# ariloytynoja/pagan2-msa

Measured on AMD Instinct MI355X. Metric: DP cells/sec, 32x100 kb DNA progressive align (hot path in dependency order: fill + traceback per tree level), higher is better.
Workload: dtype f64; 1 GPU; cfg4_32x100kb_dna_anchored; leaves=32, length=100000, data_type=dna, anchors=prefix, offset 15, node_alignments=31, order=guide-tree levels one after the other (a parent needs its children)

## Files before the change

include/pagan_dp.h:

```cpp
#ifndef PAGAN_DP_H
#define PAGAN_DP_H

#include <stdint.h>

#ifdef __cplusplus
extern "C" {
#endif

#define PAGAN_OK              0
#define PAGAN_E_ARG          -1
#define PAGAN_E_GRAPH        -2
#define PAGAN_E_BAND         -3
#define PAGAN_E_MODEL        -4
#define PAGAN_E_NODEVICE     -5
#define PAGAN_E_NOMEM        -6
#define PAGAN_E_INTERNAL     -7
#define PAGAN_DP_REACHED      0
#define PAGAN_DP_UNREACHABLE  1

#define PAGAN_OPT_NO_TERMINAL_EDGES        1u
#define PAGAN_OPT_NO_REDUCED_TERMINAL_PEN  2u

enum { PAGAN_X_MAT = 0, PAGAN_Y_MAT = 1, PAGAN_M_MAT = 2 };
enum { PAGAN_MATCHED = 2, PAGAN_XGAPPED = 3, PAGAN_YGAPPED = 4,
// ... 99 lines not shown
int  pagan_dp_debug_strips(const pagan_graph *left, const pagan_graph *right, const pagan_band *band, int32_t max_sites,
                           int32_t *strips , int32_t cap, int64_t *desc_off ,
                           int64_t *desc , int64_t desc_cap);
int  pagan_dp_debug_tiles(const pagan_graph *left, const pagan_graph *right, const pagan_band *band,
                          int32_t *tiles , int32_t cap, int32_t *tile_side);
int  pagan_dp_debug_tiles_staircase(const int32_t *tiles, int32_t n);
int  pagan_dp_debug_compact(const pagan_graph *left, const pagan_graph *right, const pagan_band *band, int32_t *keep_left,
                            int32_t *keep_right, int32_t *slot_left, int32_t *slot_right, int32_t *upper, int32_t *lower,
                            int32_t *n_out);
int  pagan_dp_debug_route(const pagan_graph *left, const pagan_graph *right, const pagan_model *model, const pagan_band *band,
                          int32_t *n_out);
int  pagan_batch_debug_scores(pagan_batch *b, int32_t k, double *dst, int64_t count);
int  pagan_batch_debug_backptrs(pagan_batch *b, int32_t k, uint32_t *dst, int64_t count);
int  pagan_batch_debug_poison(pagan_batch *b);
int  pagan_batch_debug_followed(pagan_batch *b, int32_t k, int32_t *counts);
int  pagan_batch_debug_poke_bp(pagan_batch *b, int32_t k, int32_t i, int32_t j, int32_t vit, uint32_t word);
int  pagan_batch_debug_reruns(pagan_batch *b);

void    pagan_dp_release_cache(void);
int64_t pagan_dp_cached_device_bytes(int32_t device);

typedef struct pagan_model_prob {
    int32_t      n_states;
    const float *score;
    float        gap_open;
    float        gap_ext;
    float        non_gap;
} pagan_model_prob;

typedef struct pagan_fb pagan_fb;
// ... 66 lines not shown
```

pagan2-msa_amd/__init__.py:

```python
import ctypes as C
import os

from . import abi
from .abi import Band, Graph, Model, ModelProb, Result

_HERE = os.path.dirname(os.path.abspath(__file__))
LIB_PATH = os.environ.get("PAGAN_DP_LIB") or os.path.join(_HERE, "libpagan_dp.so")
_lib = None


class PaganError(RuntimeError):
    def __init__(self, code, what):
        super().__init__("%s failed with code %d" % (what, code))
        self.code = code


def lib():
    global _lib
    if _lib is None:
        if not os.path.exists(LIB_PATH):
            raise RuntimeError("libpagan_dp.so is missing: run `python -c 'import __graft_entry__ as g; g.build()'`")
        _lib = abi.declare(C.CDLL(LIB_PATH))
    return _lib

# ... 514 lines not shown
               "pagan_batch_debug_scores")
        return out

    def debug_backptrs(self, k):
        import numpy as np
        out = np.empty((self.cells_of(k), 3), np.uint32)
        _check(self._L.pagan_batch_debug_backptrs(self._h, k, out.ctypes.data_as(C.POINTER(C.c_uint32)), out.size),
               "pagan_batch_debug_backptrs")
        return out

    def debug_followed(self, k):
        c = (C.c_int32 * 2)()
        _check(self._L.pagan_batch_debug_followed(self._h, k, c), "pagan_batch_debug_followed")
        return int(c[0]), int(c[1])

    def debug_poke_bp(self, k, i, j, vit, word):
        _check(self._L.pagan_batch_debug_poke_bp(self._h, k, i, j, vit, word), "pagan_batch_debug_poke_bp")

    def debug_reruns(self):
        return int(self._L.pagan_batch_debug_reruns(self._h))

    def debug_trace(self, k, n_cells):
        import numpy as np
        out = np.empty((n_cells, 3), np.int32)
        _check(self._L.pagan_batch_debug_trace(self._h, k, out.ctypes.data_as(C.c_void_p), out.nbytes), "pagan_batch_debug_trace")
        return out

    def debug_segments(self, k):
        import numpy as np
        info = np.zeros(4, np.int32)
# ... 22 lines not shown
```

pagan2-msa_amd/abi.py:

```python
import ctypes as C

import numpy as np

PAGAN_OK = 0
PAGAN_E_ARG, PAGAN_E_GRAPH, PAGAN_E_BAND, PAGAN_E_MODEL = -1, -2, -3, -4
PAGAN_E_NODEVICE, PAGAN_E_NOMEM, PAGAN_E_INTERNAL = -5, -6, -7
PAGAN_DP_REACHED, PAGAN_DP_UNREACHABLE = 0, 1
OPT_NO_TERMINAL_EDGES = 1
OPT_NO_REDUCED_TERMINAL_PEN = 2
SAMPLE_NO_TRACES = 1
DECODE_KEEP_MATRIX = 1
X_MAT, Y_MAT, M_MAT = 0, 1, 2
MATCHED, XGAPPED, YGAPPED, XSKIPPED, YSKIPPED = 2, 3, 4, 5, 6

_i32p = C.POINTER(C.c_int32)
_f32p = C.POINTER(C.c_float)


class CGraph(C.Structure):
    _fields_ = [("n_sites", C.c_int32), ("n_edges", C.c_int32), ("state", _i32p), ("bwd_off", _i32p),
                ("bwd_src", _i32p), ("bwd_logw", _f32p), ("bwd_eid", _i32p)]


class CModel(C.Structure):
# ... 167 lines not shown
    lib.pagan_dp_debug_strips.restype = C.c_int
    lib.pagan_dp_debug_tiles.argtypes = [gp, gp, bp, _i32p, C.c_int32, _i32p]
    lib.pagan_dp_debug_tiles.restype = C.c_int
    lib.pagan_dp_debug_compact.argtypes = [gp, gp, bp, _i32p, _i32p, _i32p, _i32p, _i32p, _i32p, _i32p]
    lib.pagan_dp_debug_compact.restype = C.c_int
    lib.pagan_dp_debug_tiles_staircase.argtypes = [_i32p, C.c_int32]
    lib.pagan_dp_debug_tiles_staircase.restype = C.c_int
    lib.pagan_dp_debug_route.argtypes = [gp, gp, C.POINTER(CModel), bp, _i32p]
    lib.pagan_dp_debug_route.restype = C.c_int
    lib.pagan_batch_debug_scores.argtypes = [C.c_void_p, C.c_int32, C.POINTER(C.c_double), C.c_int64]
    lib.pagan_batch_debug_scores.restype = C.c_int
    lib.pagan_batch_debug_backptrs.argtypes = [C.c_void_p, C.c_int32, C.POINTER(C.c_uint32), C.c_int64]
    lib.pagan_batch_debug_backptrs.restype = C.c_int
    lib.pagan_batch_debug_followed.argtypes = [C.c_void_p, C.c_int32, C.POINTER(C.c_int32)]
    lib.pagan_batch_debug_followed.restype = C.c_int
    lib.pagan_batch_debug_poke_bp.argtypes = [C.c_void_p, C.c_int32, C.c_int32, C.c_int32, C.c_int32, C.c_uint32]
    lib.pagan_batch_debug_poke_bp.restype = C.c_int
    lib.pagan_batch_debug_reruns.argtypes = [C.c_void_p]
    lib.pagan_batch_debug_reruns.restype = C.c_int
    lib.pagan_batch_debug_poison.argtypes = [C.c_void_p]
    lib.pagan_batch_debug_poison.restype = C.c_int
    lib.pagan_dp_release_cache.argtypes = []
    lib.pagan_dp_release_cache.restype = None
    lib.pagan_dp_cached_device_bytes.argtypes = [C.c_int32]
    lib.pagan_dp_cached_device_bytes.restype = C.c_int64
    mpp, f64p = C.POINTER(CModelProb), C.POINTER(C.c_double)
    lib.pagan_fb_run.argtypes = [gp, gp, mpp, bp, op, C.POINTER(C.c_void_p)]
    lib.pagan_fb_run.restype = C.c_int
    lib.pagan_fb_run_batch.argtypes = [C.c_int32, C.POINTER(gp), C.POINTER(gp), C.POINTER(mpp), C.POINTER(bp), op, C.POINTER(C.c_void_p)]
    lib.pagan_fb_run_batch.restype = C.c_int
# ... 66 lines not shown
    lib.pagan_fb_debug_decode_route.restype = C.c_int
    lib.pagan_fb_decode_predict_bytes.argtypes = [C.c_int32, C.c_int32, bp]
    lib.pagan_fb_decode_predict_bytes.restype = C.c_int64
    lib.pagan_fb_decoded_destroy.argtypes = [C.c_void_p]
    lib.pagan_fb_decoded_destroy.restype = None
    lib.pagan_fb_destroy.argtypes = [C.c_void_p]
    lib.pagan_fb_destroy.restype = None
    lib.pagan_dp_version.argtypes = []
    lib.pagan_dp_version.restype = C.c_char_p
    return lib


EXPORTED = ["pagan_dp_align", "pagan_dp_align_batch", "pagan_result_free", "pagan_dp_predict_bytes",
            "pagan_dp_count_cells", "pagan_dp_device_count", "pagan_dp_select_device", "pagan_batch_create",
            "pagan_batch_run", "pagan_batch_sync", "pagan_batch_fetch", "pagan_batch_last_ms",
            "pagan_batch_cells", "pagan_batch_last_ms_detail", "pagan_batch_destroy", "pagan_batch_debug_trace", "pagan_batch_debug_segments", "pagan_dp_debug_plan", "pagan_dp_debug_far", "pagan_dp_debug_strips", "pagan_dp_debug_tiles", "pagan_dp_debug_compact", "pagan_dp_debug_tiles_staircase", "pagan_dp_release_cache", "pagan_dp_cached_device_bytes", "pagan_dp_debug_route", "pagan_batch_debug_scores", "pagan_batch_debug_backptrs", "pagan_batch_debug_poison", "pagan_batch_debug_followed", "pagan_batch_debug_poke_bp", "pagan_batch_debug_reruns",
            "pagan_fb_run", "pagan_fb_run_batch", "pagan_fb_totals", "pagan_fb_kernel_ms", "pagan_fb_groups", "pagan_fb_schedule", "pagan_fb_debug_route", "pagan_fb_dump", "pagan_fb_posterior_cells", "pagan_fb_sample_path",
            "pagan_path_cells", "pagan_fb_path_support", "pagan_fb_site_marginals", "pagan_fb_site_marginals_batch", "pagan_fb_post_ms", "pagan_fb_predict_bytes", "pagan_sample_uniforms",
            "pagan_sample_uniforms_path", "pagan_fb_sample_paths_batch", "pagan_fb_sample_paths", "pagan_fb_samples_summary", "pagan_fb_samples_visited",
            "pagan_fb_samples_visited_all", "pagan_fb_samples_result", "pagan_fb_samples_ms", "pagan_fb_sample_predict_bytes", "pagan_fb_samples_destroy",
            "pagan_fb_decode_batch", "pagan_fb_decode", "pagan_fb_decoded_summary", "pagan_fb_decoded_visited", "pagan_fb_decoded_result",
            "pagan_fb_decoded_dump", "pagan_fb_decoded_ms", "pagan_fb_debug_decode_route", "pagan_fb_decode_predict_bytes", "pagan_fb_decoded_destroy",
            "pagan_fb_destroy", "pagan_dp_version"]
```

pagan2-msa_amd/csrc/dp_abi.hip:

```cpp
#include <hip/hip_runtime.h>

#include <algorithm>
#include <atomic>
#include <thread>
#include <chrono>
#include <cmath>
#include <cstdint>
#include <cstdio>
#include <cstdlib>
#include <cstring>
#include <condition_variable>
#include <mutex>
#include <new>
#include <type_traits>
#include <vector>
#include <unordered_map>

#include "host_anchors.h"
#include "host_graph.h"
#include "../../include/pagan_dp.h"
#include "dp_device.h"
#include "dp_band.h"

template <int BLOCK> __global__ void pg_fill_wavefront(const PgDevJob *jobs, const int *which, unsigned flags);
// ... 966 lines not shown
    d->segs = c.take<int>(6 * (size_t)(2 * hj.n_bound + 8));
}
constexpr size_t kEndStride = 64;
void carve_ends(Carver &c, int n, PgDevJob *dj) {
    char *ends = c.take<char>(kEndStride * (size_t)n);
    for (int k = 0; k < n; ++k) {
        dj[k].endcell = reinterpret_cast<int *>(ends + kEndStride * (size_t)k);
        dj[k].endscore = reinterpret_cast<double *>(ends + kEndStride * (size_t)k + 32);
    }
}

void carve_follow(Carver &c, int n, const std::vector<HostJob> &jobs, PgDevJob *dj, size_t *begin, size_t *bytes) {
    *begin = (c.cur + 255) & ~(size_t)255;
    c.cur = *begin;
    for (int k = 0; k < n; ++k) {
        dj[k].follow = nullptr; dj[k].bp_done = nullptr;
        if (jobs[k].cls.empty()) continue;
        dj[k].follow = c.take<int>(4);
        dj[k].bp_done = c.take<unsigned char>((((size_t)dj[k].nd + PG_FOLLOW_CHUNK - 1) / PG_FOLLOW_CHUNK + 15) & ~(size_t)15);
    }
    *bytes = c.cur - *begin;
}

struct StagePool {
    std::mutex m;
    std::vector<std::pair<char *, size_t>> idle;
    char *take(size_t n, size_t *cap) {
        {
            std::lock_guard<std::mutex> g(m);
            for (size_t k = 0; k < idle.size(); ++k)
                if (idle[k].second >= n) {
                    char *p = idle[k].first; *cap = idle[k].second;
                    idle.erase(idle.begin() + k);
                    return p;
// ... 83 lines not shown
        static std::atomic<bool> lds_set_dev[64];
        std::atomic<bool> &lds_set = lds_set_dev[b->device & 63];
        if (!lds_set.load()) {
            HIP_TRY(hipFuncSetAttribute(reinterpret_cast<const void *>(pg_fill_ring<true>),
                                        hipFuncAttributeMaxDynamicSharedMemorySize, (int)pg_ring_lds_bytes()));
            HIP_TRY(hipFuncSetAttribute(reinterpret_cast<const void *>(pg_fill_ring<false>),
                                        hipFuncAttributeMaxDynamicSharedMemorySize, (int)pg_ring_lds_bytes()));
            lds_set.store(true);
        }
        const int n_small = b->n_ring_small, n_big = b->n_ring - b->n_ring_small;
        HIP_TRY(hipEventRecord(b->evk[0], b->stream)); b->evk_set[0] = true;
        if (b->use_pipe) {
            bool follow = b->bp_pass == 1 && b->follow_bytes > 0 && !b->no_follow;
            if (const char *f = std::getenv("PAGAN_DP_FOLLOW")) follow = follow && std::strcmp(f, "0") != 0;
            if (b->follow_bytes > 0) HIP_TRY(hipMemsetAsync(b->arena.dev + b->follow_begin, 0, b->follow_bytes, b->stream));
            auto followers = [&](int n_fill) { return follow && n_fill <= 32 ? std::min(96, 48 * ((n_fill + 7) / 8)) : 0; };
            if (n_small > 0)
                hipLaunchKernelGGL((pg_fill_pipe<true, false>), dim3(n_small + followers(n_small)), dim3(pg_pipe_block()), 0 , b->stream,
                                   b->d_jobs, b->d_which, b->flags | chk_banded, n_small);
            if (n_big > 0)
                hipLaunchKernelGGL((pg_fill_pipe<false, false>), dim3(n_big + followers(n_big)), dim3(pg_pipe_block()), 0, b->stream,
                                   b->d_jobs, b->d_which + n_small, b->flags | chk_banded, n_big);
            HIP_TRY(hipEventRecord(b->evk[1], b->stream)); b->evk_set[1] = true;
            if (b->bp_pass) {
                int max_nd = 1, max_w = 1;
                for (int k = 0; k < b->n; ++k) if (b->jobs[k].ring_ok) { max_nd = std::max(max_nd, b->dj[k].nd); max_w = std::max(max_w, b->jobs[k].dx.max_width); }
                const int zc = (max_w + PG_BP_CELLS - 1) / PG_BP_CELLS, dpb = bp_diags_per_block(max_nd, b->n_ring * zc);
                hipLaunchKernelGGL(pg_backptr, dim3((max_nd + dpb - 1) / dpb, b->n_ring, zc), dim3(256), 0, b->stream,
                                   b->d_jobs, b->d_which, (b->flags & 0xffu) | (b->bp_pass == 2 ? 0x100u : chk_banded), dpb);
                HIP_TRY(hipEventRecord(b->evk[2], b->stream)); b->evk_set[2] = true;
            }
        } else {
            b->evk_set[1] = false;
            if (n_small > 0)
                hipLaunchKernelGGL(pg_fill_ring<true>, dim3(n_small), dim3(576), pg_ring_lds_bytes(), b->stream,
                                   b->d_jobs, b->d_which, b->flags);
            if (n_big > 0)
// ... 688 lines not shown
    });
    const double tc3 = now();
    b->trace_off.resize(n); b->end_off.resize(n); b->score_off.resize(n);
    char *base = b->arena.dev;
    auto rebase = [&](auto *&p) { p = reinterpret_cast<std::remove_reference_t<decltype(p)>>(base + reinterpret_cast<size_t>(p)); };
    for (int k = 0; k < n; ++k) {
        PgDevJob &d = b->dj[k];
        b->trace_off[k] = reinterpret_cast<size_t>(d.trace);
        b->end_off[k] = reinterpret_cast<size_t>(d.endcell);
        b->score_off[k] = reinterpret_cast<size_t>(d.endscore);
        rebase(d.stL); rebase(d.offL); rebase(d.srcL); rebase(d.lwL);
        rebase(d.stR); rebase(d.offR); rebase(d.srcR); rebase(d.lwR);
        rebase(d.table); rebase(d.imin); rebase(d.imax); rebase(d.doff); rebase(d.tb); rebase(d.dsc); if (d.psc) { rebase(d.psc); rebase(d.sched); } if (d.hfL) { rebase(d.hfL); rebase(d.hfR); } rebase(d.fill_status);
        rebase(d.sc); rebase(d.bp);
        rebase(d.trace); rebase(d.endcell); rebase(d.endscore); rebase(d.segs); rebase(d.ttab);
        if (d.follow) { rebase(d.follow); rebase(d.bp_done); }
    }
    for (size_t g = 0; g < sdev.size(); ++g) {
        const StripPlan &sp = b->jobs[sdev[g].job].strips[sdev[g].q];
        PgDevJob d = b->dj[sdev[g].job];
        d.psc = reinterpret_cast<int *>(base + reinterpret_cast<size_t>(sdev[g].psc)) - 8 * (ptrdiff_t)sp.d0;
        d.sched = reinterpret_cast<int *>(base + reinterpret_cast<size_t>(sdev[g].sched));
        d.follow = reinterpret_cast<int *>(base + reinterpret_cast<size_t>(sdev[g].follow));
        d.bp_done = nullptr;
        d.nd = sp.d1;
        d.is_strip = 1; d.strip_row0 = sp.r0; d.d_first = sp.d0; d.feed_wave = sp.feed_wave; d.col_first = sp.col_first;
        d.pdsc = b->dj[sdev[g].job].dsc;
        d.prev_follow = nullptr; d.prev_nd = 0;
        if (sdev[g].q > 0) {
            d.prev_follow = b->dj[(size_t)n + g - 1].follow;
            d.prev_nd = b->dj[(size_t)n + g - 1].nd;
        }
        b->dj[(size_t)n + g] = d;
    }
    std::memcpy(stage.data() + reinterpret_cast<size_t>(jobs_off), b->dj.data(), sizeof(PgDevJob) * b->dj.size());
    std::memcpy(stage.data() + reinterpret_cast<size_t>(which_off), which_ring.data(), sizeof(int) * n);
    if (!swhich.empty()) std::memcpy(stage.data() + reinterpret_cast<size_t>(swhich_off), swhich.data(), sizeof(int) * swhich.size());
    b->d_swhich = reinterpret_cast<int *>(base + reinterpret_cast<size_t>(swhich_off));
    b->d_jobs = reinterpret_cast<PgDevJob *>(base + reinterpret_cast<size_t>(jobs_off));
// ... 243 lines not shown
int pagan_batch_debug_reruns(pagan_batch *b) { return b ? b->reruns : PAGAN_E_ARG; }

int pagan_batch_debug_followed(pagan_batch *b, int32_t k, int32_t *counts) {
    if (!b || k < 0 || k >= b->n || !counts) return PAGAN_E_ARG;
    counts[0] = counts[1] = 0;
    if (!b->dj[k].bp_done) return PAGAN_OK;
    HIP_TRY(hipStreamSynchronize(b->stream));
    const size_t n = ((size_t)b->dj[k].nd + PG_FOLLOW_CHUNK - 1) / PG_FOLLOW_CHUNK;
    std::vector<unsigned char> flags(n);
    HIP_TRY(hipMemcpy(flags.data(), b->dj[k].bp_done, n, hipMemcpyDeviceToHost));
    counts[1] = (int32_t)n;
    for (unsigned char f : flags) counts[0] += f != 0;
    return PAGAN_OK;
}

int pagan_batch_debug_scores(pagan_batch *b, int32_t k, double *dst, int64_t count) {
    if (!b || k < 0 || k >= b->n || !dst || count > 3 * b->jobs[k].dx.cells) return PAGAN_E_ARG;
    HIP_TRY(hipStreamSynchronize(b->stream));
    HIP_TRY(hipMemcpy(dst, b->dj[k].sc, sizeof(double) * (size_t)count, hipMemcpyDeviceToHost));
    return PAGAN_OK;
}

int pagan_batch_debug_backptrs(pagan_batch *b, int32_t k, uint32_t *dst, int64_t count) {
    if (!b || k < 0 || k >= b->n || !dst || count > 3 * b->jobs[k].dx.cells) return PAGAN_E_ARG;
    HIP_TRY(hipStreamSynchronize(b->stream));
    HIP_TRY(hipMemcpy(dst, b->dj[k].bp, sizeof(uint32_t) * (size_t)count, hipMemcpyDeviceToHost));
    return PAGAN_OK;
}

int pagan_batch_debug_trace(pagan_batch *b, int32_t k, void *dst, int64_t bytes) {
// ... 122 lines not shown
```

pagan2-msa_amd/csrc/dp_device.h:

```cpp
#pragma once
#include <stdint.h>

#define PG_BP_NONE 3u
#define PG_BP_ADJL 4u
#define PG_BP_ADJR 8u
#define PG_MAX_SLOT 16383
#define PG_SEG 256
#define PG_BP_DIAGS 64
#define PG_BP_CELLS 1024
#define PG_STATUS_PATH_CHECK 3
#define PG_FLAG_SCORE_CHECK 0x200u
#define PG_FLAG_STRIPS_SPREAD 0x10000u
#define PG_FILL_SCORE_MISMATCH 0x7c
#define PG_FILL_OTHER_XCD 0x20000000
#define PG_FOLLOW_CHUNK 16

#define PG_PIPE_WIDTH 242
#define PG_PIPE_REACH 14
#define PG_PIPE_RING 14
#define PG_HIST_SLOTS 3
#define PG_HIST_MAX_SPAN 44
#define PG_PIPE_ASSIST 3
#define PG_PIPE_STAGE 3
#define PG_PIPE_WAKE 6
#define PG_PIPE_WINDOW 432
#define PG_PIPE_WINDOW_A 352
#define PG_PIPE_EDGE_CAP 1024
#define PG_PIPE_SITE_EDGES 126

#define PG_TILE 64
// ... 14 lines not shown
    const int *sched;
    const unsigned char *hfL, *hfR;
    int *fill_status;
    long long cells;
    double *sc;
    unsigned *bp;
    int *trace;
    int *endcell;
    double *endscore;
    int n_bound;
    const int *tb;
    int *ttab;
    int *segs;
    int *follow;
    unsigned char *bp_done;
    int is_strip;
    int strip_row0;
    int d_first;
    int feed_wave;
    int col_first;
    int prev_nd;
    const int *prev_follow;
    const int *pdsc;
};
#ifndef PG_STRIP_ROWS
#define PG_STRIP_ROWS 192
#endif
#define PG_STRIP_TERM 8
```

pagan2-msa_amd/csrc/dp_kernels.hip:

```cpp
#include <hip/hip_runtime.h>
#include "dp_device.h"

#include "dp_kcommon.h"


template <int BLOCK>
__global__ __launch_bounds__(BLOCK) void pg_fill_wavefront(const PgDevJob *__restrict__ jobs,
                                                           const int *__restrict__ which, unsigned flags) {
    const View J = load_view(jobs + which[blockIdx.x]);
    const bool no_terminal_edges = flags & 1u;
    const bool reduced_terminal = !(flags & 2u);
    Diag d1 = {0, -1, 0}, d2 = {0, -1, 0};
    for (int d = 0; d < J.nd; ++d) {
        const int lo = J.imin[d], hi = J.imax[d];
        const long long base = J.doff[d];
        for (int i = lo + (int)threadIdx.x; i <= hi; i += BLOCK)
            fill_cell_hbm(J, d, d1, d2, i, d - i, base + (i - lo), no_terminal_edges, reduced_terminal);
        d2 = d1;
        d1 = {lo, hi, base};
        __syncthreads();
    }
}

template __global__ void pg_fill_wavefront<64>(const PgDevJob *, const int *, unsigned);
// ... 365 lines not shown
                }
            } else if (!all_by_gap) {
                SM.sc[d & (RK - 1)][u][PG_M] = bm;
                if (active) { orow[PG_M] = bm; brow[PG_M] = pm; }
            }
            resident |= slot_bit;
        }
        if ((d & (RK / 2 - 1)) == 0) asm volatile("s_waitcnt vmcnt(0)" ::: "memory");
        lds_barrier();
    }
}

template __global__ void pg_fill_ring<true>(const PgDevJob *, const int *, unsigned);
template __global__ void pg_fill_ring<false>(const PgDevJob *, const int *, unsigned);

namespace {

struct TNode { int i, j, vit; };

__device__ __forceinline__ bool trace_done(const TNode &n) { return n.i < 1 && n.j < 1; }

struct TCache { int d0 = -1000; pg_i4 a, b, c; };
__device__ __forceinline__ bool trace_step(const View &J, TNode &n, int &w, TCache &C) {
    if (n.vit < 0 || n.vit > 2 || n.i < 0 || n.j < 0 || n.i >= J.Lx || n.j >= J.Ly) return false;
    const int dd = n.i + n.j;
    PG_GLOBAL const pg_i4 *gd = (PG_GLOBAL const pg_i4 *)(unsigned long long)J.dsc;
    const int back = C.d0 - dd;
    pg_i4 D;
    if (back == 0) { D = C.a; }
    else if (back == 1) { D = C.b; C.a = C.b; C.b = C.c; C.c = gd[dd >= 2 ? dd - 2 : 0]; C.d0 = dd; }
    else if (back == 2) { D = C.c; C.a = C.c; C.b = gd[dd >= 1 ? dd - 1 : 0]; C.c = gd[dd >= 2 ? dd - 2 : 0]; C.d0 = dd; }
    else { D = gd[dd]; C.a = D; C.b = gd[dd >= 1 ? dd - 1 : 0]; C.c = gd[dd >= 2 ? dd - 2 : 0]; C.d0 = dd; }
    const int mn = D.x, mx = D.y;
    if (n.i < mn || n.i > mx) return false;
    const long long ix = (((long long)D.w << 32) | (unsigned)D.z) + (n.i - mn);
    const int oL = J.offL[n.i], oR = J.offR[n.j];
    const unsigned b = J.bp[3 * ix + n.vit];
    w = (int)((unsigned)n.vit | (b & ~3u));
    const unsigned from = b & 3u;
    if (from == PG_BP_NONE) return false;
    const int k1 = (int)((b >> 4) & 16383u), k2 = (int)(b >> 18);
    if (n.vit != PG_Y) n.i = (b & PG_BP_ADJL) ? n.i - 1 : J.srcL[oL + k1];
    if (n.vit != PG_X) n.j = (b & PG_BP_ADJR) ? n.j - 1 : J.srcR[oR + k2];
    n.vit = (int)from;
    return true;
}

__device__ __forceinline__ int boundary_of(int d, int K) {
    if (d <= 0) return 0;
    int k = 0;
    if (d % PG_SEG == 0) k = d / PG_SEG; else if ((d + 1) % PG_SEG == 0) k = (d + 1) / PG_SEG;
    return (k >= 1 && k <= K) ? k : 0;
}

__device__ __forceinline__ int entry_index(const View &J, int k, const TNode &n) {
    const int D = k * PG_SEG, dd = n.i + n.j;
    if (dd == D) return 3 * (n.i - J.imin[D]) + n.vit;
    const int w = J.imax[D] - J.imin[D] + 1;
    return 3 * (w > 0 ? w : 0) + 3 * (n.i - J.imin[D - 1]) + n.vit;
}

enum { EXIT_ENTRY = 0, EXIT_MISS = 1, EXIT_DONE = 2 };

}

__global__ void pg_end_corner(const PgDevJob *__restrict__ jobs, const int *__restrict__ tiles_gave_up) {
    if (threadIdx.x != 0) return;
    const View J = load_view(jobs + blockIdx.x);
    const double NI = neg_inf();
    const Diag none = {0, -1, 0};
    const int Lx = J.Lx, Ly = J.Ly;
    const int l0 = J.offL[Lx], l1 = J.offL[Lx + 1];
    const int r0 = J.offR[Ly], r1 = J.offR[Ly + 1];

    double best = NI;
    int mat = -1, xi = -1, yi = -1, kl = -1, kr = -1;
    if (l1 > l0 && r1 > r0) {
        const double ng = (double)J.ng;
        auto m_cand = [&](int e1, int e2) {
            const int p = J.srcL[e1], q = J.srcR[e2];
// ... 22 lines not shown
        }
    }
    J.endscore[0] = best;
    gint_w ec = J.endcell;
    ec[1] = mat; ec[2] = xi; ec[3] = yi; ec[4] = kl; ec[5] = kr; ec[6] = 0; ec[7] = 0;
    ec[0] = (best > NI) ? 0 : 1;
    if (jobs[blockIdx.x].fill_status[0] != 0) ec[0] = 0x40000000 | jobs[blockIdx.x].fill_status[0];
    else if (tiles_gave_up && tiles_gave_up[0] != 0) ec[0] = 0x40000000 | 0x7e;
}

__global__ __launch_bounds__(128) void pg_trace_spec(const PgDevJob *__restrict__ jobs) {
    const View J = load_view(jobs + blockIdx.y);
    if (J.n_bound < 1 || J.endcell[0] != 0) return;
    const int eg = (int)(blockIdx.x * blockDim.x + threadIdx.x);
    if (eg >= J.tb[J.n_bound + 1]) return;
    int k = 1;
    for (int hi = J.n_bound; k < hi;) { const int mid = (k + hi + 1) >> 1; if (J.tb[mid] <= eg) k = mid; else hi = mid - 1; }
    const int D = k * PG_SEG;
    const int mnA = J.imin[D], wA = max(J.imax[D] - mnA + 1, 0);
    const int mnB = J.imin[D - 1], wB = max(J.imax[D - 1] - mnB + 1, 0);
    const int n_entries = 3 * (wA + wB);
    gint_w tab = J.ttab + 8 * (long long)J.tb[k];
    {
        const int e = eg - J.tb[k];
        if (e >= n_entries) return;
        TNode n;
        if (e < 3 * wA) { n.i = mnA + e / 3; n.j = D - n.i; } else { n.i = mnB + (e - 3 * wA) / 3; n.j = D - 1 - n.i; }
        n.vit = e % 3;
        int steps = 0, kind = EXIT_DONE, w;
        bool ok = true;
        TCache tc;
        const bool follow = n_entries <= 3 * 512;
        int kb = k - 1, low = (k - 1) * PG_SEG;
        for (;;) {
            if (trace_done(n)) { kind = EXIT_DONE; break; }
            const int dd = n.i + n.j;
            if (steps > 0 && kb >= 1 && dd <= low) {
                if (dd >= low - 1) { kind = EXIT_ENTRY; break; }
                if (!follow) { kind = EXIT_MISS; break; }
                while (kb >= 1 && dd < low - 1) { --kb; low -= PG_SEG; }
                if (kb >= 1 && dd <= low) { kind = EXIT_ENTRY; break; }
            }
            if (steps >= 2 * PG_SEG) { kind = EXIT_MISS; break; }
            if (!trace_step(J, n, w, tc)) { ok = false; break; }
            ++steps;
        }
        int next = -1;
        if (ok && kind == EXIT_ENTRY && n.vit >= 0 && n.vit <= 2) {
            const int dd = n.i + n.j, mn = J.imin[dd], mx = J.imax[dd];
            if (n.i >= mn && n.i <= mx) next = J.tb[kb] + entry_index(J, kb, n);
        }
        typedef int i4 __attribute__((ext_vector_type(4)));
        i4 a; a.x = n.i; a.y = n.j; a.z = (n.vit & 3) | (kind << 2); a.w = ok ? steps : -1;
        i4 b; b.x = next; b.y = 0; b.z = 0; b.w = 0;
        *(PG_GLOBAL i4 *)(tab + 8 * e) = a;
        *(PG_GLOBAL i4 *)(tab + 8 * e + 4) = b;
    }
}

__global__ void pg_trace_compose(const PgDevJob *__restrict__ jobs) {
    if (threadIdx.x != 0) return;
    const View J = load_view(jobs + blockIdx.x);
    gint_w ec = J.endcell;
    if (ec[0] != 0) return;
    TNode n; n.vit = ec[1]; n.i = ec[2]; n.j = ec[3];
    const int cap = J.Lx + J.Ly, seg_cap = 2 * J.n_bound + 8;
    int off = 0, nseg = 0, status = 0;
    gint_w tr = J.trace;
    long long cur = -1;
    TCache tc;
    while (!trace_done(n)) {
        if (off >= cap) { status = 2; break; }
// ... 99 lines not shown
```

pagan2-msa_amd/csrc/dp_pipe.hip:

```cpp
#include "dp_kcommon.h"
#include <type_traits>

#define PNW 4
#define PNT (64 * PNW)
#define PNTW PG_PIPE_WIDTH
#define PRK PG_PIPE_RING
#define PAGE PG_PIPE_REACH
#define PRW 512
#define PEC PG_PIPE_EDGE_CAP
#define PDR 128
#define PDR_REACH 60
#define PLOOK 64
#define PLAND 8
#define PNA PG_PIPE_ASSIST
#define PST PG_PIPE_STAGE
#define PBLOCK (PNT + 64 * PNA + 64)
static_assert(PNTW == PNT - PAGE && PRK >= PAGE && PG_PIPE_WINDOW + 80 <= PRW, "kernel geometry out of step with dp_device.h");
static_assert(PNA == 3 && PST == 3 && PAGE >= PLAND + 4, "assist wave a stages the diagonals d % 3 == a into slot a, at most two diagonals ahead; far cells have landed");
#define PFAR_POOL ((PNT * 4) / 24)
#define PS_ONLY 0x80000000u
#define PS_FIRST 0x40000000u
#define PS_BP 0x3fffffffu
#ifndef PG_SPIN_LIMIT_LOG2
#define PG_SPIN_LIMIT_LOG2 25
// ... 2648 lines not shown
                     [&](int k, int &p, double &lw) { p = J.srcL[l0 + k]; lw = (double)J.lwL[l0 + k]; },
                     [&](int k, int &q, double &rw) { q = J.srcR[r0 + k]; rw = (double)J.lwR[r0 + k]; },
                     bx, by, bm, px, py, pm);
            typedef unsigned u3 __attribute__((ext_vector_type(3)));
            u3 b; b.x = px; b.y = py; b.z = pm;
            *(PG_GLOBAL u3 *)(J.bp + 3 * at) = b;
            if (flags & PG_FLAG_SCORE_CHECK) {
                double sx, sy, sm_;
                far_cell((PG_GLOBAL const double *)(J.sc + 3 * at), sx, sy, sm_);
                const bool same = __double_as_longlong(bx) == __double_as_longlong(sx) && __double_as_longlong(by) == __double_as_longlong(sy) &&
                                  __double_as_longlong(bm) == __double_as_longlong(sm_);
                if (!same) report_fill_status(job, PG_FILL_SCORE_MISMATCH);
            }
        }
    }
    if (lane == 0) ((PG_GLOBAL unsigned char *)job->bp_done)[chunk] = 1;
}

__device__ __noinline__ void pipe_follower(const PgDevJob *__restrict__ jobs, const int *__restrict__ which, int n_fill, unsigned flags) {
    const int lane = threadIdx.x & 63;
    const unsigned xcc = my_xcc_id();
    int mine[4], n_mine = 0;
    for (int w = (int)(blockIdx.x & 7u); w < n_fill && n_mine < 4; w += 8) {
        const PgDevJob *__restrict__ job = jobs + which[w];
        if (!job->follow) continue;
        int id = 0;
        for (int spin = 0; spin < 20000 && (id = peek_l2((PG_GLOBAL const int *)job->follow + 1)) == 0; ++spin) __builtin_amdgcn_s_sleep(32);
        if (id == (int)xcc + 1) mine[n_mine++] = which[w];
    }
    unsigned left = (1u << n_mine) - 1u;
    int idle = 0;
    const int start = (int)(threadIdx.x >> 6);
    while (left != 0 && idle < 200000) {
        bool worked = false;
        for (int t = 0; t < n_mine; ++t) {
            const int k = (t + start) % n_mine;
            if (!(left & (1u << k))) continue;
            const PgDevJob *__restrict__ job = jobs + mine[k];
            PG_GLOBAL int *fw = (PG_GLOBAL int *)job->follow;
            const int nd = job->nd, n_chunks = (nd + PG_FOLLOW_CHUNK - 1) / PG_FOLLOW_CHUNK;
            const int next = peek_l2(fw + 2);
            if (next >= n_chunks) { left &= ~(1u << k); continue; }
            const int chk = (flags & PG_FLAG_SCORE_CHECK) ? 1 : 0;
            const int last = ((next + 1) * PG_FOLLOW_CHUNK - 1 < nd - 1 ? (next + 1) * PG_FOLLOW_CHUNK - 1 : nd - 1) + chk;
            if (peek_l2(fw) < last) continue;
            int c = 0;
            if (lane == 0) c = __hip_atomic_fetch_add(fw + 2, 1, __ATOMIC_RELAXED, __HIP_MEMORY_SCOPE_AGENT);
            c = __builtin_amdgcn_readfirstlane(c);
            if (c >= n_chunks) { left &= ~(1u << k); continue; }
            const int lastc = ((c + 1) * PG_FOLLOW_CHUNK - 1 < nd - 1 ? (c + 1) * PG_FOLLOW_CHUNK - 1 : nd - 1) + chk;
            int spin = 0;
            while (peek_l2(fw) < lastc && spin < 200000) { __builtin_amdgcn_s_sleep(32); ++spin; }
            if (spin >= 200000) return;
            follow_chunk(job, c, lane, flags);
            worked = true;
        }
        if (worked) idle = 0; else { __builtin_amdgcn_s_sleep(64); ++idle; }
    }
}

#define PHALO 16
#define PFEED 32
static_assert(PHALO >= PAGE - 1 && 64 / PHALO * 8 == PFEED, "feeder geometry");
__device__ __noinline__ void strip_feeder(const PgDevJob *__restrict__ job, cdesc8_p psc, int tid, int wave, unsigned flags) {
    const int lane = tid & 63;
    wave = __builtin_amdgcn_readfirstlane(wave);
    const int nd = job->nd, d0 = job->d_first;
    const int hq = lane / PHALO, hr = lane % PHALO;
    const int row = job->strip_row0 - PHALO + hr;
    const int col = row & (PNT - 1);
    const int dn = (wave + 1) % PNW;
    PG_GLOBAL const int *prev = (PG_GLOBAL const int *)job->prev_follow;
// ... 518 lines not shown
```

Measured before the change: 605.2 million cells/s.

## Overlap boundary traceback with fill using follower waves and a contiguous-chunk watermark

Follower waves in the fill kernel now also run the per-boundary traceback entries once the backpointer chunks a boundary depends on are complete. A contiguous-done watermark is kept over bp_done, and per-boundary completion counters are added. The later traceback kernel skips boundaries already marked done, so traceback work overlaps the fill instead of running after it. This adds atomics, L2-coherent loads and a few extra arena buffers, and the follower waves keep spinning for longer. The trace code moves into a shared header.

```diff
diff --git a/include/pagan_dp.h b/include/pagan_dp.h
--- a/include/pagan_dp.h
+++ b/include/pagan_dp.h
@@ -137,6 +137,8 @@
 int  pagan_batch_debug_backptrs(pagan_batch *b, int32_t k, uint32_t *dst, int64_t count);
 int  pagan_batch_debug_poison(pagan_batch *b);
 int  pagan_batch_debug_followed(pagan_batch *b, int32_t k, int32_t *counts);
+int  pagan_batch_debug_traced(pagan_batch *b, int32_t k, int32_t *counts);
+int  pagan_dp_debug_boundary_chunk(int32_t k, int32_t info[2]);
 int  pagan_batch_debug_poke_bp(pagan_batch *b, int32_t k, int32_t i, int32_t j, int32_t vit, uint32_t word);
 int  pagan_batch_debug_reruns(pagan_batch *b);
 
diff --git a/pagan2-msa_amd/__init__.py b/pagan2-msa_amd/__init__.py
--- a/pagan2-msa_amd/__init__.py
+++ b/pagan2-msa_amd/__init__.py
@@ -552,6 +552,11 @@
         _check(self._L.pagan_batch_debug_followed(self._h, k, c), "pagan_batch_debug_followed")
         return int(c[0]), int(c[1])
 
+    def debug_traced(self, k):
+        c = (C.c_int32 * 2)()
+        _check(self._L.pagan_batch_debug_traced(self._h, k, c), "pagan_batch_debug_traced")
+        return int(c[0]), int(c[1])
+
     def debug_poke_bp(self, k, i, j, vit, word):
         _check(self._L.pagan_batch_debug_poke_bp(self._h, k, i, j, vit, word), "pagan_batch_debug_poke_bp")
 
diff --git a/pagan2-msa_amd/abi.py b/pagan2-msa_amd/abi.py
--- a/pagan2-msa_amd/abi.py
+++ b/pagan2-msa_amd/abi.py
@@ -205,6 +205,10 @@
     lib.pagan_batch_debug_backptrs.restype = C.c_int
     lib.pagan_batch_debug_followed.argtypes = [C.c_void_p, C.c_int32, C.POINTER(C.c_int32)]
     lib.pagan_batch_debug_followed.restype = C.c_int
+    lib.pagan_batch_debug_traced.argtypes = [C.c_void_p, C.c_int32, C.POINTER(C.c_int32)]
+    lib.pagan_batch_debug_traced.restype = C.c_int
+    lib.pagan_dp_debug_boundary_chunk.argtypes = [C.c_int32, _i32p]
+    lib.pagan_dp_debug_boundary_chunk.restype = C.c_int
     lib.pagan_batch_debug_poke_bp.argtypes = [C.c_void_p, C.c_int32, C.c_int32, C.c_int32, C.c_int32, C.c_uint32]
     lib.pagan_batch_debug_poke_bp.restype = C.c_int
     lib.pagan_batch_debug_reruns.argtypes = [C.c_void_p]
@@ -301,7 +305,7 @@
 EXPORTED = ["pagan_dp_align", "pagan_dp_align_batch", "pagan_result_free", "pagan_dp_predict_bytes",
             "pagan_dp_count_cells", "pagan_dp_device_count", "pagan_dp_select_device", "pagan_batch_create",
             "pagan_batch_run", "pagan_batch_sync", "pagan_batch_fetch", "pagan_batch_last_ms",
-            "pagan_batch_cells", "pagan_batch_last_ms_detail", "pagan_batch_destroy", "pagan_batch_debug_trace", "pagan_batch_debug_segments", "pagan_dp_debug_plan", "pagan_dp_debug_far", "pagan_dp_debug_strips", "pagan_dp_debug_tiles", "pagan_dp_debug_compact", "pagan_dp_debug_tiles_staircase", "pagan_dp_release_cache", "pagan_dp_cached_device_bytes", "pagan_dp_debug_route", "pagan_batch_debug_scores", "pagan_batch_debug_backptrs", "pagan_batch_debug_poison", "pagan_batch_debug_followed", "pagan_batch_debug_poke_bp", "pagan_batch_debug_reruns",
+            "pagan_batch_cells", "pagan_batch_last_ms_detail", "pagan_batch_destroy", "pagan_batch_debug_trace", "pagan_batch_debug_segments", "pagan_dp_debug_plan", "pagan_dp_debug_far", "pagan_dp_debug_strips", "pagan_dp_debug_tiles", "pagan_dp_debug_compact", "pagan_dp_debug_tiles_staircase", "pagan_dp_release_cache", "pagan_dp_cached_device_bytes", "pagan_dp_debug_route", "pagan_batch_debug_scores", "pagan_batch_debug_backptrs", "pagan_batch_debug_poison", "pagan_batch_debug_followed", "pagan_batch_debug_traced", "pagan_dp_debug_boundary_chunk", "pagan_batch_debug_poke_bp", "pagan_batch_debug_reruns",
             "pagan_fb_run", "pagan_fb_run_batch", "pagan_fb_totals", "pagan_fb_kernel_ms", "pagan_fb_groups", "pagan_fb_schedule", "pagan_fb_debug_route", "pagan_fb_dump", "pagan_fb_posterior_cells", "pagan_fb_sample_path",
             "pagan_path_cells", "pagan_fb_path_support", "pagan_fb_site_marginals", "pagan_fb_site_marginals_batch", "pagan_fb_post_ms", "pagan_fb_predict_bytes", "pagan_sample_uniforms",
             "pagan_sample_uniforms_path", "pagan_fb_sample_paths_batch", "pagan_fb_sample_paths", "pagan_fb_samples_summary", "pagan_fb_samples_visited",
diff --git a/pagan2-msa_amd/csrc/dp_abi.hip b/pagan2-msa_amd/csrc/dp_abi.hip
--- a/pagan2-msa_amd/csrc/dp_abi.hip
+++ b/pagan2-msa_amd/csrc/dp_abi.hip
@@ -1004,10 +1004,12 @@
     *begin = (c.cur + 255) & ~(size_t)255;
     c.cur = *begin;
     for (int k = 0; k < n; ++k) {
-        dj[k].follow = nullptr; dj[k].bp_done = nullptr;
+        dj[k].follow = nullptr; dj[k].bp_done = nullptr; dj[k].tr_count = nullptr; dj[k].tr_done = nullptr;
         if (jobs[k].cls.empty()) continue;
-        dj[k].follow = c.take<int>(4);
+        dj[k].follow = c.take<int>(8);
         dj[k].bp_done = c.take<unsigned char>((((size_t)dj[k].nd + PG_FOLLOW_CHUNK - 1) / PG_FOLLOW_CHUNK + 15) & ~(size_t)15);
+        dj[k].tr_count = c.take<int>((size_t)jobs[k].n_bound + 1);
+        dj[k].tr_done = c.take<unsigned char>((size_t)jobs[k].n_bound + 1);
     }
     *bytes = c.cur - *begin;
 }
@@ -1121,13 +1123,16 @@
             bool follow = b->bp_pass == 1 && b->follow_bytes > 0 && !b->no_follow;
             if (const char *f = std::getenv("PAGAN_DP_FOLLOW")) follow = follow && std::strcmp(f, "0") != 0;
             if (b->follow_bytes > 0) HIP_TRY(hipMemsetAsync(b->arena.dev + b->follow_begin, 0, b->follow_bytes, b->stream));
+            bool trace_follow = follow && !(b->poke[0] >= 0 && b->poke[0] < b->n);
+            if (const char *f = std::getenv("PAGAN_DP_TRACE_FOLLOW")) trace_follow = trace_follow && std::strcmp(f, "0") != 0;
+            const unsigned tf = trace_follow ? PG_FLAG_TRACE_FOLLOW : 0u;
             auto followers = [&](int n_fill) { return follow && n_fill <= 32 ? std::min(96, 48 * ((n_fill + 7) / 8)) : 0; };
             if (n_small > 0)
                 hipLaunchKernelGGL((pg_fill_pipe<true, false>), dim3(n_small + followers(n_small)), dim3(pg_pipe_block()), 0 , b->stream,
-                                   b->d_jobs, b->d_which, b->flags | chk_banded, n_small);
+                                   b->d_jobs, b->d_which, (b->flags & ~PG_FLAG_TRACE_FOLLOW) | chk_banded | tf, n_small);
             if (n_big > 0)
                 hipLaunchKernelGGL((pg_fill_pipe<false, false>), dim3(n_big + followers(n_big)), dim3(pg_pipe_block()), 0, b->stream,
-                                   b->d_jobs, b->d_which + n_small, b->flags | chk_banded, n_big);
+                                   b->d_jobs, b->d_which + n_small, (b->flags & ~PG_FLAG_TRACE_FOLLOW) | chk_banded | tf, n_big);
             HIP_TRY(hipEventRecord(b->evk[1], b->stream)); b->evk_set[1] = true;
             if (b->bp_pass) {
                 int max_nd = 1, max_w = 1;
@@ -1846,7 +1851,7 @@
         rebase(d.table); rebase(d.imin); rebase(d.imax); rebase(d.doff); rebase(d.tb); rebase(d.dsc); if (d.psc) { rebase(d.psc); rebase(d.sched); } if (d.hfL) { rebase(d.hfL); rebase(d.hfR); } rebase(d.fill_status);
         rebase(d.sc); rebase(d.bp);
         rebase(d.trace); rebase(d.endcell); rebase(d.endscore); rebase(d.segs); rebase(d.ttab);
-        if (d.follow) { rebase(d.follow); rebase(d.bp_done); }
+        if (d.follow) { rebase(d.follow); rebase(d.bp_done); rebase(d.tr_count); rebase(d.tr_done); }
     }
     for (size_t g = 0; g < sdev.size(); ++g) {
         const StripPlan &sp = b->jobs[sdev[g].job].strips[sdev[g].q];
@@ -1854,7 +1859,7 @@
         d.psc = reinterpret_cast<int *>(base + reinterpret_cast<size_t>(sdev[g].psc)) - 8 * (ptrdiff_t)sp.d0;
         d.sched = reinterpret_cast<int *>(base + reinterpret_cast<size_t>(sdev[g].sched));
         d.follow = reinterpret_cast<int *>(base + reinterpret_cast<size_t>(sdev[g].follow));
-        d.bp_done = nullptr;
+        d.bp_done = nullptr; d.tr_count = nullptr; d.tr_done = nullptr;
         d.nd = sp.d1;
         d.is_strip = 1; d.strip_row0 = sp.r0; d.d_first = sp.d0; d.feed_wave = sp.feed_wave; d.col_first = sp.col_first;
         d.pdsc = b->dj[sdev[g].job].dsc;
@@ -2128,6 +2133,22 @@
     return PAGAN_OK;
 }
 
+int pagan_batch_debug_traced(pagan_batch *b, int32_t k, int32_t *counts) {
+    if (!b || k < 0 || k >= b->n || !counts) return PAGAN_E_ARG;
+    counts[0] = 0; counts[1] = b->jobs[k].n_bound;
+    if (!b->dj[k].tr_done || b->jobs[k].n_bound < 1) return PAGAN_OK;
+    HIP_TRY(hipStreamSynchronize(b->stream));
+    std::vector<unsigned char> flags((size_t)b->jobs[k].n_bound + 1);
+    HIP_TRY(hipMemcpy(flags.data(), b->dj[k].tr_done, flags.size(), hipMemcpyDeviceToHost));
+    for (size_t q = 1; q < flags.size(); ++q) counts[0] += flags[q] != 0;
+    return PAGAN_OK;
+}
+
+int pagan_dp_debug_boundary_chunk(int32_t k, int32_t info[2]) {
+    if (info) { info[0] = PG_SEG; info[1] = PG_FOLLOW_CHUNK; }
+    return k >= 1 ? pg_boundary_chunk(k) : PAGAN_E_ARG;
+}
+
 int pagan_batch_debug_scores(pagan_batch *b, int32_t k, double *dst, int64_t count) {
     if (!b || k < 0 || k >= b->n || !dst || count > 3 * b->jobs[k].dx.cells) return PAGAN_E_ARG;
     HIP_TRY(hipStreamSynchronize(b->stream));
diff --git a/pagan2-msa_amd/csrc/dp_device.h b/pagan2-msa_amd/csrc/dp_device.h
--- a/pagan2-msa_amd/csrc/dp_device.h
+++ b/pagan2-msa_amd/csrc/dp_device.h
@@ -14,6 +14,13 @@
 #define PG_FILL_SCORE_MISMATCH 0x7c
 #define PG_FILL_OTHER_XCD 0x20000000
 #define PG_FOLLOW_CHUNK 16
+#define PG_FLAG_TRACE_FOLLOW 0x20000u
+#define PG_TRACE_PIECE 64
+
+#ifdef __HIPCC__
+__host__ __device__
+#endif
+static inline int pg_boundary_chunk(int k) { return (int)(((long long)k * PG_SEG) / PG_FOLLOW_CHUNK); }
 
 #define PG_PIPE_WIDTH 242
 #define PG_PIPE_REACH 14
@@ -58,6 +65,8 @@
     int *segs;
     int *follow;
     unsigned char *bp_done;
+    int *tr_count;
+    unsigned char *tr_done;
     int is_strip;
     int strip_row0;
     int d_first;
diff --git a/pagan2-msa_amd/csrc/dp_kernels.hip b/pagan2-msa_amd/csrc/dp_kernels.hip
--- a/pagan2-msa_amd/csrc/dp_kernels.hip
+++ b/pagan2-msa_amd/csrc/dp_kernels.hip
@@ -2,7 +2,7 @@
 #include "dp_device.h"
 
 #include "dp_kcommon.h"
-
+#include "dp_trace.h"
 
 template <int BLOCK>
 __global__ __launch_bounds__(BLOCK) void pg_fill_wavefront(const PgDevJob *__restrict__ jobs,
@@ -403,56 +403,6 @@
 template __global__ void pg_fill_ring<true>(const PgDevJob *, const int *, unsigned);
 template __global__ void pg_fill_ring<false>(const PgDevJob *, const int *, unsigned);
 
-namespace {
-
-struct TNode { int i, j, vit; };
-
-__device__ __forceinline__ bool trace_done(const TNode &n) { return n.i < 1 && n.j < 1; }
-
-struct TCache { int d0 = -1000; pg_i4 a, b, c; };
-__device__ __forceinline__ bool trace_step(const View &J, TNode &n, int &w, TCache &C) {
-    if (n.vit < 0 || n.vit > 2 || n.i < 0 || n.j < 0 || n.i >= J.Lx || n.j >= J.Ly) return false;
-    const int dd = n.i + n.j;
-    PG_GLOBAL const pg_i4 *gd = (PG_GLOBAL const pg_i4 *)(unsigned long long)J.dsc;
-    const int back = C.d0 - dd;
-    pg_i4 D;
-    if (back == 0) { D = C.a; }
-    else if (back == 1) { D = C.b; C.a = C.b; C.b = C.c; C.c = gd[dd >= 2 ? dd - 2 : 0]; C.d0 = dd; }
-    else if (back == 2) { D = C.c; C.a = C.c; C.b = gd[dd >= 1 ? dd - 1 : 0]; C.c = gd[dd >= 2 ? dd - 2 : 0]; C.d0 = dd; }
-    else { D = gd[dd]; C.a = D; C.b = gd[dd >= 1 ? dd - 1 : 0]; C.c = gd[dd >= 2 ? dd - 2 : 0]; C.d0 = dd; }
-    const int mn = D.x, mx = D.y;
-    if (n.i < mn || n.i > mx) return false;
-    const long long ix = (((long long)D.w << 32) | (unsigned)D.z) + (n.i - mn);
-    const int oL = J.offL[n.i], oR = J.offR[n.j];
-    const unsigned b = J.bp[3 * ix + n.vit];
-    w = (int)((unsigned)n.vit | (b & ~3u));
-    const unsigned from = b & 3u;
-    if (from == PG_BP_NONE) return false;
-    const int k1 = (int)((b >> 4) & 16383u), k2 = (int)(b >> 18);
-    if (n.vit != PG_Y) n.i = (b & PG_BP_ADJL) ? n.i - 1 : J.srcL[oL + k1];
-    if (n.vit != PG_X) n.j = (b & PG_BP_ADJR) ? n.j - 1 : J.srcR[oR + k2];
-    n.vit = (int)from;
-    return true;
-}
-
-__device__ __forceinline__ int boundary_of(int d, int K) {
-    if (d <= 0) return 0;
-    int k = 0;
-    if (d % PG_SEG == 0) k = d / PG_SEG; else if ((d + 1) % PG_SEG == 0) k = (d + 1) / PG_SEG;
-    return (k >= 1 && k <= K) ? k : 0;
-}
-
-__device__ __forceinline__ int entry_index(const View &J, int k, const TNode &n) {
-    const int D = k * PG_SEG, dd = n.i + n.j;
-    if (dd == D) return 3 * (n.i - J.imin[D]) + n.vit;
-    const int w = J.imax[D] - J.imin[D] + 1;
-    return 3 * (w > 0 ? w : 0) + 3 * (n.i - J.imin[D - 1]) + n.vit;
-}
-
-enum { EXIT_ENTRY = 0, EXIT_MISS = 1, EXIT_DONE = 2 };
-
-}
-
 __global__ void pg_end_corner(const PgDevJob *__restrict__ jobs, const int *__restrict__ tiles_gave_up) {
     if (threadIdx.x != 0) return;
     const View J = load_view(jobs + blockIdx.x);
@@ -505,48 +455,10 @@
     if (J.n_bound < 1 || J.endcell[0] != 0) return;
     const int eg = (int)(blockIdx.x * blockDim.x + threadIdx.x);
     if (eg >= J.tb[J.n_bound + 1]) return;
-    int k = 1;
-    for (int hi = J.n_bound; k < hi;) { const int mid = (k + hi + 1) >> 1; if (J.tb[mid] <= eg) k = mid; else hi = mid - 1; }
-    const int D = k * PG_SEG;
-    const int mnA = J.imin[D], wA = max(J.imax[D] - mnA + 1, 0);
-    const int mnB = J.imin[D - 1], wB = max(J.imax[D - 1] - mnB + 1, 0);
-    const int n_entries = 3 * (wA + wB);
-    gint_w tab = J.ttab + 8 * (long long)J.tb[k];
-    {
-        const int e = eg - J.tb[k];
-        if (e >= n_entries) return;
-        TNode n;
-        if (e < 3 * wA) { n.i = mnA + e / 3; n.j = D - n.i; } else { n.i = mnB + (e - 3 * wA) / 3; n.j = D - 1 - n.i; }
-        n.vit = e % 3;
-        int steps = 0, kind = EXIT_DONE, w;
-        bool ok = true;
-        TCache tc;
-        const bool follow = n_entries <= 3 * 512;
-        int kb = k - 1, low = (k - 1) * PG_SEG;
-        for (;;) {
-            if (trace_done(n)) { kind = EXIT_DONE; break; }
-            const int dd = n.i + n.j;
-            if (steps > 0 && kb >= 1 && dd <= low) {
-                if (dd >= low - 1) { kind = EXIT_ENTRY; break; }
-                if (!follow) { kind = EXIT_MISS; break; }
-                while (kb >= 1 && dd < low - 1) { --kb; low -= PG_SEG; }
-                if (kb >= 1 && dd <= low) { kind = EXIT_ENTRY; break; }
-            }
-            if (steps >= 2 * PG_SEG) { kind = EXIT_MISS; break; }
-            if (!trace_step(J, n, w, tc)) { ok = false; break; }
-            ++steps;
-        }
-        int next = -1;
-        if (ok && kind == EXIT_ENTRY && n.vit >= 0 && n.vit <= 2) {
-            const int dd = n.i + n.j, mn = J.imin[dd], mx = J.imax[dd];
-            if (n.i >= mn && n.i <= mx) next = J.tb[kb] + entry_index(J, kb, n);
-        }
-        typedef int i4 __attribute__((ext_vector_type(4)));
-        i4 a; a.x = n.i; a.y = n.j; a.z = (n.vit & 3) | (kind << 2); a.w = ok ? steps : -1;
-        i4 b; b.x = next; b.y = 0; b.z = 0; b.w = 0;
-        *(PG_GLOBAL i4 *)(tab + 8 * e) = a;
-        *(PG_GLOBAL i4 *)(tab + 8 * e + 4) = b;
-    }
+    const int k = boundary_of_entry(J, eg);
+    PG_GLOBAL const unsigned char *done = (PG_GLOBAL const unsigned char *)jobs[blockIdx.y].tr_done;
+    if (done && done[k]) return;
+    trace_entry<false>(J, k, eg);
 }
 
 __global__ void pg_trace_compose(const PgDevJob *__restrict__ jobs) {
diff --git a/pagan2-msa_amd/csrc/dp_pipe.hip b/pagan2-msa_amd/csrc/dp_pipe.hip
--- a/pagan2-msa_amd/csrc/dp_pipe.hip
+++ b/pagan2-msa_amd/csrc/dp_pipe.hip
@@ -1,4 +1,5 @@
 #include "dp_kcommon.h"
+#include "dp_trace.h"
 #include <type_traits>
 
 #define PNW 4
@@ -2686,7 +2687,59 @@
             }
         }
     }
+    asm volatile("s_waitcnt vmcnt(0)" ::: "memory");
     if (lane == 0) ((PG_GLOBAL unsigned char *)job->bp_done)[chunk] = 1;
+}
+
+__device__ __forceinline__ int peek_l2_u8(PG_GLOBAL const unsigned char *p) {
+    int v;
+    asm volatile("global_load_ubyte %0, %1, off sc1\n\ts_waitcnt vmcnt(0)" : "=&v"(v) : "v"(p) : "memory");
+    return v;
+}
+
+__device__ __forceinline__ void raise_watermark(const PgDevJob *__restrict__ job, int n_chunks, int lane) {
+    PG_GLOBAL int *fw = (PG_GLOBAL int *)job->follow;
+    PG_GLOBAL const unsigned char *done = (PG_GLOBAL const unsigned char *)job->bp_done;
+    asm volatile("s_waitcnt vmcnt(0)" ::: "memory");
+    const int wm0 = peek_l2(fw + 3);
+    int wm = wm0;
+    while (wm < n_chunks) {
+        const int c = wm + lane;
+        int v = 0;
+        if (c < n_chunks) v = peek_l2_u8(done + c);
+        const unsigned long long set = __ballot(v != 0);
+        const int run = ~set == 0ull ? 64 : __builtin_ctzll(~set);
+        wm += run;
+        if (run < 64) break;
+    }
+    if (wm > n_chunks) wm = n_chunks;
+    if (lane == 0 && wm > wm0) __hip_atomic_fetch_max(fw + 3, wm, __ATOMIC_RELAXED, __HIP_MEMORY_SCOPE_AGENT);
+}
+
+__device__ __noinline__ void trace_piece(const PgDevJob *__restrict__ job, int piece, int lane) {
+    const View J = load_view(job);
+    const int total = J.tb[J.n_bound + 1];
+    const int eg = piece * PG_TRACE_PIECE + lane;
+    const bool valid = eg < total;
+    int k = 0;
+    if (valid) {
+        k = boundary_of_entry(J, eg);
+        trace_entry<true>(J, k, eg);
+    }
+    PG_GLOBAL int *count = (PG_GLOBAL int *)job->tr_count;
+    PG_GLOBAL unsigned char *done = (PG_GLOBAL unsigned char *)job->tr_done;
+    unsigned long long todo = __ballot(valid);
+    while (todo != 0) {
+        const int src = __builtin_ctzll(todo);
+        const int kk = __builtin_amdgcn_readlane(k, src);
+        const unsigned long long same = __ballot(valid && k == kk);
+        if (lane == src) {
+            const int n = __builtin_popcountll(same);
+            const int before = __hip_atomic_fetch_add(count + kk, n, __ATOMIC_RELAXED, __HIP_MEMORY_SCOPE_AGENT);
+            if (before + n == J.tb[kk + 1] - J.tb[kk]) done[kk] = 1;
+        }
+        todo &= ~same;
+    }
 }
 
 __device__ __noinline__ void pipe_follower(const PgDevJob *__restrict__ jobs, const int *__restrict__ which, int n_fill, unsigned flags) {
@@ -2701,9 +2754,10 @@
         if (id == (int)xcc + 1) mine[n_mine++] = which[w];
     }
     unsigned left = (1u << n_mine) - 1u;
-    int idle = 0;
+    unsigned left_tr = (flags & PG_FLAG_TRACE_FOLLOW) ? left : 0u;
+    int idle = 0, idle_tr = 0;
     const int start = (int)(threadIdx.x >> 6);
-    while (left != 0 && idle < 200000) {
+    while ((left | left_tr) != 0 && idle < 200000) {
         bool worked = false;
         for (int t = 0; t < n_mine; ++t) {
             const int k = (t + start) % n_mine;
@@ -2725,9 +2779,37 @@
             while (peek_l2(fw) < lastc && spin < 200000) { __builtin_amdgcn_s_sleep(32); ++spin; }
             if (spin >= 200000) return;
             follow_chunk(job, c, lane, flags);
+            if (flags & PG_FLAG_TRACE_FOLLOW) raise_watermark(job, n_chunks, lane);
             worked = true;
         }
-        if (worked) idle = 0; else { __builtin_amdgcn_s_sleep(64); ++idle; }
+        for (int t = 0; t < n_mine && !worked; ++t) {
+            const int k = (t + start) % n_mine;
+            if (!(left_tr & (1u << k))) continue;
+            const PgDevJob *__restrict__ job = jobs + mine[k];
+            PG_GLOBAL int *fw = (PG_GLOBAL int *)job->follow;
+            const int K = job->n_bound;
+            const int total = (K >= 1 && job->tr_done) ? job->tb[K + 1] : 0, n_pieces = (total + PG_TRACE_PIECE - 1) / PG_TRACE_PIECE;
+            const int next = peek_l2(fw + 4);
+            if (next >= n_pieces) { left_tr &= ~(1u << k); continue; }
+            const int last_entry = (next + 1) * PG_TRACE_PIECE - 1 < total - 1 ? (next + 1) * PG_TRACE_PIECE - 1 : total - 1;
+            int kh = 1;
+            for (int hi = K; kh < hi;) { const int mid = (kh + hi + 1) >> 1; if (job->tb[mid] <= last_entry) kh = mid; else hi = mid - 1; }
+            if (peek_l2(fw + 3) <= pg_boundary_chunk(kh)) continue;
+            int got = 0;
+            if (lane == 0) {
+                int expected = next;
+                got = __hip_atomic_compare_exchange_strong(fw + 4, &expected, next + 1, __ATOMIC_RELAXED, __ATOMIC_RELAXED, __HIP_MEMORY_SCOPE_AGENT) ? 1 : 0;
+            }
+            if (__builtin_amdgcn_readfirstlane(got) == 0) continue;
+            trace_piece(job, next, lane);
+            worked = true;
+        }
+        if (worked) { idle = 0; idle_tr = 0; }
+        else {
+            __builtin_amdgcn_s_sleep(64);
+            ++idle;
+            if (left == 0 && ++idle_tr > 4000) left_tr = 0;
+        }
     }
 }
 
diff --git a/pagan2-msa_amd/csrc/dp_trace.h b/pagan2-msa_amd/csrc/dp_trace.h
--- /dev/null
+++ b/pagan2-msa_amd/csrc/dp_trace.h
@@ -0,0 +1,101 @@
+#pragma once
+#include "dp_kcommon.h"
+
+namespace {
+
+struct TNode { int i, j, vit; };
+
+__device__ __forceinline__ bool trace_done(const TNode &n) { return n.i < 1 && n.j < 1; }
+
+struct TCache { int d0 = -1000; pg_i4 a, b, c; };
+template <bool L2 = false>
+__device__ __forceinline__ bool trace_step(const View &J, TNode &n, int &w, TCache &C) {
+    if (n.vit < 0 || n.vit > 2 || n.i < 0 || n.j < 0 || n.i >= J.Lx || n.j >= J.Ly) return false;
+    const int dd = n.i + n.j;
+    PG_GLOBAL const pg_i4 *gd = (PG_GLOBAL const pg_i4 *)(unsigned long long)J.dsc;
+    const int back = C.d0 - dd;
+    pg_i4 D;
+    if (back == 0) { D = C.a; }
+    else if (back == 1) { D = C.b; C.a = C.b; C.b = C.c; C.c = gd[dd >= 2 ? dd - 2 : 0]; C.d0 = dd; }
+    else if (back == 2) { D = C.c; C.a = C.c; C.b = gd[dd >= 1 ? dd - 1 : 0]; C.c = gd[dd >= 2 ? dd - 2 : 0]; C.d0 = dd; }
+    else { D = gd[dd]; C.a = D; C.b = gd[dd >= 1 ? dd - 1 : 0]; C.c = gd[dd >= 2 ? dd - 2 : 0]; C.d0 = dd; }
+    const int mn = D.x, mx = D.y;
+    if (n.i < mn || n.i > mx) return false;
+    const long long ix = (((long long)D.w << 32) | (unsigned)D.z) + (n.i - mn);
+    const int oL = J.offL[n.i], oR = J.offR[n.j];
+    const unsigned b = L2 ? __hip_atomic_load(J.bp + (3 * ix + n.vit), __ATOMIC_RELAXED, __HIP_MEMORY_SCOPE_AGENT) : J.bp[3 * ix + n.vit];
+    w = (int)((unsigned)n.vit | (b & ~3u));
+    const unsigned from = b & 3u;
+    if (from == PG_BP_NONE) return false;
+    const int k1 = (int)((b >> 4) & 16383u), k2 = (int)(b >> 18);
+    if (n.vit != PG_Y) n.i = (b & PG_BP_ADJL) ? n.i - 1 : J.srcL[oL + k1];
+    if (n.vit != PG_X) n.j = (b & PG_BP_ADJR) ? n.j - 1 : J.srcR[oR + k2];
+    n.vit = (int)from;
+    return true;
+}
+
+__device__ __forceinline__ int boundary_of(int d, int K) {
+    if (d <= 0) return 0;
+    int k = 0;
+    if (d % PG_SEG == 0) k = d / PG_SEG; else if ((d + 1) % PG_SEG == 0) k = (d + 1) / PG_SEG;
+    return (k >= 1 && k <= K) ? k : 0;
+}
+
+__device__ __forceinline__ int entry_index(const View &J, int k, const TNode &n) {
+    const int D = k * PG_SEG, dd = n.i + n.j;
+    if (dd == D) return 3 * (n.i - J.imin[D]) + n.vit;
+    const int w = J.imax[D] - J.imin[D] + 1;
+    return 3 * (w > 0 ? w : 0) + 3 * (n.i - J.imin[D - 1]) + n.vit;
+}
+
+enum { EXIT_ENTRY = 0, EXIT_MISS = 1, EXIT_DONE = 2 };
+
+__device__ __forceinline__ int boundary_of_entry(const View &J, int eg) {
+    int k = 1;
+    for (int hi = J.n_bound; k < hi;) { const int mid = (k + hi + 1) >> 1; if (J.tb[mid] <= eg) k = mid; else hi = mid - 1; }
+    return k;
+}
+
+template <bool L2>
+__device__ __forceinline__ void trace_entry(const View &J, int k, int eg) {
+    const int D = k * PG_SEG;
+    const int mnA = J.imin[D], wA = max(J.imax[D] - mnA + 1, 0);
+    const int mnB = J.imin[D - 1], wB = max(J.imax[D - 1] - mnB + 1, 0);
+    const int n_entries = 3 * (wA + wB);
+    gint_w tab = J.ttab + 8 * (long long)J.tb[k];
+    const int e = eg - J.tb[k];
+    if (e >= n_entries) return;
+    TNode n;
+    if (e < 3 * wA) { n.i = mnA + e / 3; n.j = D - n.i; } else { n.i = mnB + (e - 3 * wA) / 3; n.j = D - 1 - n.i; }
+    n.vit = e % 3;
+    int steps = 0, kind = EXIT_DONE, w;
+    bool ok = true;
+    TCache tc;
+    const bool follow = n_entries <= 3 * 512;
+    int kb = k - 1, low = (k - 1) * PG_SEG;
+    for (;;) {
+        if (trace_done(n)) { kind = EXIT_DONE; break; }
+        const int dd = n.i + n.j;
+        if (steps > 0 && kb >= 1 && dd <= low) {
+            if (dd >= low - 1) { kind = EXIT_ENTRY; break; }
+            if (!follow) { kind = EXIT_MISS; break; }
+            while (kb >= 1 && dd < low - 1) { --kb; low -= PG_SEG; }
+            if (kb >= 1 && dd <= low) { kind = EXIT_ENTRY; break; }
+        }
+        if (steps >= 2 * PG_SEG) { kind = EXIT_MISS; break; }
+        if (!trace_step<L2>(J, n, w, tc)) { ok = false; break; }
+        ++steps;
+    }
+    int next = -1;
+    if (ok && kind == EXIT_ENTRY && n.vit >= 0 && n.vit <= 2) {
+        const int dd = n.i + n.j, mn = J.imin[dd], mx = J.imax[dd];
+        if (n.i >= mn && n.i <= mx) next = J.tb[kb] + entry_index(J, kb, n);
+    }
+    typedef int i4 __attribute__((ext_vector_type(4)));
+    i4 a; a.x = n.i; a.y = n.j; a.z = (n.vit & 3) | (kind << 2); a.w = ok ? steps : -1;
+    i4 b; b.x = next; b.y = 0; b.z = 0; b.w = 0;
+    *(PG_GLOBAL i4 *)(tab + 8 * e) = a;
+    *(PG_GLOBAL i4 *)(tab + 8 * e + 4) = b;
+}
+
+}
```

Measured after the change: 609.5 million cells/s, median of 6. Within noise of the previous version (+0.7%).
